# AER-RC/RRTMG_LW

Measured on AMD Instinct MI355X. Metric: columns/sec, 72-layer profiles, higher is better.
Workload: dtype f64 (transmittance / tfn codes and their LDS table f32); 1 GPU; 1000000 synthetic 72-layer columns, config 'cloudy' (icld=2: rtrnmr max-random overlap, idrv=0), sharded 1x1000000; ncol_total=1000000, nlay=72, columns_per_gpu=1000000, parallelism=columns/1, gather=none, kdata=stand-in (real k-data absent from the reference mount), sweeps=production

## Files before the change

rrtmg_lw_amd/csrc/driver.hip:

```cpp
#include <hip/hip_runtime.h>
#include <cstdlib>
#include <sched.h>

#include <algorithm>
#include <array>
#include <atomic>
#include <cstdint>
#include <cstdarg>
#include <mutex>
#include <string>
#include <chrono>
#include <condition_variable>
#include <functional>
#include <map>
#include <thread>
#include <type_traits>
#include <vector>

#include "../../include/rrtmg_lw_hip.h"
#include "kernels.hip"
#include "mtjump.hpp"
#include "hostrows.hpp"
#include "owned.hpp"

// ... 336 lines not shown

int launches_ok()
{
    const hipError_t e = hipGetLastError();
    if (e != hipSuccess) return fail(RRTMG_LW_HIP_EHIP, "kernel launch failed: %s", hipGetErrorString(e));
    return 0;
}

#ifdef RRLW_TUNE
constexpr bool TUNING = true;
#else
constexpr bool TUNING = false;
#endif
constexpr bool sweepc_exists(int phase, bool ddt) { return !ddt || (!TUNING && phase != 1); }
constexpr bool sweepc_ddt(int phase, int idrv) { return idrv == 1 && phase != 1; }
constexpr bool sweepz_exists(int mode, bool ddt) { return !TUNING || (mode == 2 && !ddt); }
constexpr bool layer_exists(bool gcm, int cloud) { return TUNING ? gcm && cloud == 1 : gcm || cloud != 3; }

constexpr int EVERY = -1;
template <int... Vs, class F>
int with_const(int v, F &&f)
{
    int rc = 0;
    bool hit = false;
    ((((v == Vs || v == EVERY) && rc == 0) ? (void)(hit = true, rc = f(std::integral_constant<int, Vs>{})) : (void)0), ...);
    return hit ? rc : fail(RRTMG_LW_HIP_EARG, "internal: no kernel instantiation for %d", v);
}

struct KernelName { char s[24]; };
constexpr KernelName sweep_name(char family, int nq, int x, bool spec)
{
    KernelName n{};
    int k = 0;
    for (const char *p = "k_sweep"; *p; p++) n.s[k++] = *p;
    n.s[k++] = family; n.s[k++] = '<'; n.s[k++] = (char)('0' + nq); n.s[k++] = ','; n.s[k++] = (char)('0' + x);
    if (spec) for (const char *p = ",spec"; *p; p++) n.s[k++] = *p;
    n.s[k++] = '>';
    return n;
}
template <int Q, int PH, bool I, bool SPEC>
struct SweepC {
    static constexpr KernelName name = sweep_name('c', Q, PH, SPEC);
    static constexpr int nt = sweepc_nt(Q, PH);
    static constexpr auto kernel() { return &k_sweepc<Q, PH, I, nt, SPEC>; }
    static int nsb(int nbands) { return sweepc_nsb(Q, PH, I, nbands); }
    static int lds_bytes(int wnb, int nsb) { return sweepc_lds_bytes(PH, I, wnb, nsb, nt); }
};
template <int Q, int M, bool I, bool SPEC>
struct SweepZ {
    static constexpr KernelName name = sweep_name('z', Q, M, SPEC);
    static constexpr int nt = sweepz_nt(Q);
    static constexpr auto kernel() { return &k_sweepz<Q, M, I, SPEC>; }
    static int nsb(int nbands) { return sweepz_nsb(Q, nbands, I); }
    static int lds_bytes(int wnb, int nsb) { return sweepz_lds_bytes(wnb, nsb, nt, I); }
};
template <class F>
int sweepc_dispatch(int nq, int phase, int ddt, int spec, F &&f)
{
    return with_const<1, 2, 3, 4>(nq, [&](auto Q) { return with_const<0, 1, 2>(phase, [&](auto PH) {
           return with_const<0, 1>(ddt, [&](auto I) { return with_const<0, 1>(spec, [&](auto S) {
               if constexpr (sweepc_exists(decltype(PH)::value, decltype(I)::value != 0))
                   return f(SweepC<decltype(Q)::value, decltype(PH)::value, decltype(I)::value != 0, decltype(S)::value != 0>{});
               else return ddt == EVERY ? 0 : fail(RRTMG_LW_HIP_EARG, "internal: no such k_sweepc");
           }); }); }); });
}
template <class F>
int sweepz_dispatch(int nq, int mode, int ddt, int spec, F &&f)
{
    return with_const<1, 2, 3, 4>(nq, [&](auto Q) { return with_const<1, 2, 3, 4>(mode, [&](auto M) {
           return with_const<0, 1>(ddt, [&](auto I) { return with_const<0, 1>(spec, [&](auto S) {
               if constexpr (sweepz_exists(decltype(M)::value, decltype(I)::value != 0))
                   return f(SweepZ<decltype(Q)::value, decltype(M)::value, decltype(I)::value != 0, decltype(S)::value != 0>{});
               else return ddt == EVERY ? 0 : fail(RRTMG_LW_HIP_EARG, "internal: no such k_sweepz");
           }); }); }); });
}

constexpr int N1_LDS_MAX = 160 * 1024;
int ensure_sweep_attrs()
{
    if (G.sweep_attrs) return 0;
    const auto raise = [](auto K) { HIP_TRY(hipFuncSetAttribute((const void *)K.kernel(), hipFuncAttributeMaxDynamicSharedMemorySize, SWEEPC_LDS_MAX)); return 0; };
    if (int rc = sweepc_dispatch(EVERY, EVERY, EVERY, EVERY, raise)) return rc;
    if (int rc = sweepz_dispatch(EVERY, EVERY, EVERY, EVERY, raise)) return rc;
    HIP_TRY(hipFuncSetAttribute((const void *)k_flux<false>, hipFuncAttributeMaxDynamicSharedMemorySize, FLUX_LDS_BYTES));
    HIP_TRY(hipFuncSetAttribute((const void *)k_flux<true>, hipFuncAttributeMaxDynamicSharedMemorySize, FLUX_LDS_BYTES));
#ifndef RRLW_TUNE
    HIP_TRY(hipFuncSetAttribute((const void *)k_n1<false>, hipFuncAttributeMaxDynamicSharedMemorySize, N1_LDS_MAX));
#endif
    G.sweep_attrs = true;
    return 0;
}

struct SweepGroups { int n = 0; int nb[NGROUP_MAX]; unsigned long long bands[NGROUP_MAX]; int gq[NGROUP_MAX]; };
bool make_groups(int mode, int idrv, int istart, int iend, SweepGroups &fg)
{
    unsigned long long lists[5] = {0, 0, 0, 0, 0};
    int nbs[5] = {0, 0, 0, 0, 0};
    for (int nq = 1; nq <= 4; nq++)
        for (int B = 1; B <= NBND; B++)
            if (band_nquad(B) == nq && B >= istart && B <= iend) lists[nq] |= (unsigned long long)(B - 1) << (4 * nbs[nq]++);
    fg.n = 0;
    for (int nq = 4; nq >= 1; nq--) {
        const int zcap = sweepz_group_cap(nq, idrv == 1);
        const int cap = std::max(1, std::min(sweepc_group_cap(nq), mode != 0 ? zcap : 99));
        for (int k0 = 0; k0 < nbs[nq]; k0 += cap) {
            if (fg.n >= NGROUP_MAX) return false;
            const int nbg = std::min(cap, nbs[nq] - k0);
            fg.nb[fg.n] = nbg;
            fg.bands[fg.n] = (lists[nq] >> (4 * k0)) & (nbg >= 16 ? ~0ull : ((1ull << (4 * nbg)) - 1ull));
            fg.gq[fg.n++] = nq;
        }
    }
    return true;
}

void graphs_clear();
int g_split_max = []() { const char *e = getenv("RRTMG_LW_SPLIT_MAX"); return e ? std::max(0, atoi(e)) : 768; }();
int ensure_workspace(int nlay, int ncolb, bool cloud, bool mc = false, int idrv = 1, int mode = -1)
{
    SweepGroups fgw;
    int groups = NGROUP_MAX;
    if (mode >= 0 && make_groups(mode, idrv, 1, NBND, fgw)) groups = fgw.n;
    const bool gdp = idrv == 1, efcl = cloud && (mode < 0 || mode == 1 || mode == 3), ovl = cloud && (mode < 0 || mode == 2);
    const size_t split_cols = ncolb <= g_split_max ? (size_t)NBND * align_up((size_t)ncolb, 64) : 0;
    const State::WsShape &have = G.ws;
    if (G.ws_buf && have.nlay == nlay && have.ncolb >= ncolb && (have.cloud || !cloud) && (have.mc || !mc) && (have.two_scr || !G.split_sweep) &&
        have.groups >= groups && have.slabcols >= split_cols && (have.gdp || !gdp) && (have.efcl || !efcl) && (have.ovl || !ovl)) return 0;
    if (G.ws_buf) { HIP_TRY(hipDeviceSynchronize()); graphs_clear(); if (int rc = drop(G.ws_buf, "workspace")) return rc; }
    const bool same = have.nlay == nlay;
    ncolb = std::max(ncolb, same ? have.ncolb : 0);
    cloud = cloud || have.cloud || mc;
    mc = mc || have.mc;
    const int ng = std::max(groups, have.groups);
    const bool want_gdp = gdp || have.gdp, want_efcl = efcl || have.efcl, want_ovl = ovl || have.ovl;
    const size_t n = (size_t)ncolb, L = (size_t)nlay;
    const size_t slabcols = std::max((size_t)ng * n, (size_t)NBND * align_up(std::min(n, (size_t)std::max(g_split_max, 0)), 64));
    struct Item { void **p; size_t bytes; };
    Workspace &W = G.W;
    W = Workspace{};
    std::vector<Item> items = {
        {(void **)&W.gdn1, slabcols * (L + 1) * sizeof(double)},
        {(void **)&W.gup1, slabcols * (L + 1) * sizeof(double)},
        {(void **)&W.gup, slabcols * (L + 1) * sizeof(Part2)},
        {(void **)&W.gdn, slabcols * (L + 1) * sizeof(Part2)},
    };
    if (want_gdp) items.push_back({(void **)&W.gdp, slabcols * (L + 1) * sizeof(Part2)});
    const bool two_scr = G.split_sweep;
    G.scrset[1] = State::ScrSet{};
    for (int k = 0; k < (two_scr ? 2 : 1); k++) {
        State::ScrSet &ss = G.scrset[k];
        ss = State::ScrSet{};
        items.push_back({(void **)&ss.scr[S_CODE], (size_t)NQUAD * L * n * CODE_BYTES});
        items.push_back({(void **)&ss.fw, (size_t)NFW * L * n * sizeof(unsigned)});
        if (cloud) items.push_back({(void **)&ss.scr[S_CODET], (size_t)NQUAD * L * n * CODE_BYTES});
    }
    for (auto &ps : G.prep) {
        ps = State::PrepSet{};
        items.push_back({(void **)&ps.percol, (size_t)NPERCOL * n * 8});
        items.push_back({(void **)&ps.laytrop, n * 4});
        items.push_back({(void **)&ps.ncbands, n * 4});
        items.push_back({(void **)&ps.cflag, (L + 2) * n * 4});
        const size_t nblk = (n + 63) / 64, nslot = (size_t)sort_slots((int)nblk);
        items.push_back({(void **)&ps.btop, nblk * 4});
        items.push_back({(void **)&ps.hblk, nblk * 4});
        items.push_back({(void **)&ps.order, nslot * 4});
        items.push_back({(void **)&ps.hgrp, (nslot / SORT_GROUP) * 4});
        items.push_back({(void **)&ps.bbot, nblk * 4});
        items.push_back({(void **)&ps.hbot, (nslot / SORT_GROUP) * 4});
// ... 187 lines not shown
    sa.tlev = GCM ? g.tlev : c.tz;
    if (GCM && out.uflxs) { sa.uflxs = out.uflxs; sa.dflxs = out.dflxs; sa.uflxcs = out.uflxcs; sa.dflxcs = out.dflxcs; }
    return sa;
}

template <bool GCM>
int run_sweep(hipStream_t s, const Workspace &Wk_, const Batch &b, const GcmIn &g, const ColIn &c, const FluxOut &out, int sset = 0)
{
    Workspace Wk = Wk_;
    const int nb = b.nb;
    const size_t pcb_split = align_up((size_t)nb, 64);
    const bool split = nb <= g_split_max && (size_t)NBND * pcb_split <= G.ws.slabcols && pcb_split <= (size_t)Wk.ncolb;
    Wk.pcb = split ? (int)pcb_split : Wk.ncolb;
    if (int rc = ensure_sweep_attrs()) return rc;
    const bool fan = G.sweep_fanout;
    State::SweepSet &SS = G.swset[sset];
    if (fan) {
        if (int rc = ensure_sweep_set(sset)) return rc;
        HIP_TRY(hipEventRecord(SS.go.get(), s));
        for (int k = 0; k < 3; k++) HIP_TRY(hipStreamWaitEvent(SS.q[k].get(), SS.go.get(), 0));
    }
    SweepArgs sa = sweep_args<GCM>(b, g, c, out);
    const bool spec = sa.uflxs != nullptr;
#ifndef RRLW_TUNE
    if (G.n1 && b.mode == 0 && GCM && b.istart == 1 && b.iend == 16 && b.idrv == 0 && !spec && n1_lds_bytes(b.nlay) <= N1_LDS_MAX) {
        const dim3 ngrid((nb + N1_WAVES - 1) / N1_WAVES), nblock(64 * N1_WAVES);
        LAUNCH_LDS("k_n1", (k_n1<false>), ngrid, nblock, n1_lds_bytes(b.nlay), s, G.D, Wk, sa, out, g.plev);
        return launches_ok();
    }
#endif
    sa.split = split ? 1 : 0;
    const bool cfree = g_clear_groups && b.mode != 0 && !one_sweep(nb, b.mode);
    sa.cfree = cfree ? 1 : 0;
    SweepGroups fg;
    if (!make_groups(b.mode, b.idrv, b.istart, b.iend, fg)) return fail(RRTMG_LW_HIP_EARG, "internal: more than %d sweep groups", NGROUP_MAX);
    if ((!split && fg.n > G.ws.groups) || (b.idrv == 1 && !G.ws.gdp)) return fail(RRTMG_LW_HIP_EARG, "internal: workspace holds %d band groups, the call needs %d", G.ws.groups, fg.n);
    int slab0[NGROUP_MAX];
    unsigned long long gsz = 0ull;
    { int sl = 0; for (int gi = 0; gi < fg.n; gi++) { slab0[gi] = sl; const int n = split ? fg.nb[gi] : 1; gsz |= (unsigned long long)n << (4 * gi); sl += n; } }
    hipStream_t gs = s;
    const auto launch = [&](auto K) {
        using Kn = decltype(K);
        const int wnb = split ? 1 : sa.nbands;
        const int nsb = split ? 1 : Kn::nsb(sa.nbands);
        sa.ncb = (nb + 64 * nsb - 1) / (64 * nsb);
        const dim3 sgrid((unsigned)sa.ncb, split ? sa.nbands : 1), sblock(64, wnb * Kn::nt, nsb);
        LAUNCH_LDS(Kn::name.s, Kn::kernel(), sgrid, sblock, Kn::lds_bytes(wnb, nsb), gs, G.D, Wk, sa);
        return 0;
    };
    const auto sweepc = [&](int nq, int phase) {
        if (TUNING && b.idrv == 1) return fail(RRTMG_LW_HIP_EARG, "tuning build: idrv = 0 only");
        return sweepc_dispatch(nq, phase, sweepc_ddt(phase, b.idrv), spec, launch);
    };
    const auto sweepz = [&](int nq) {
        const int zmode = b.mode == 1 ? 1 : b.mode == 3 ? (b.mc ? 3 : 4) : 2;
        if (!sweepz_exists(zmode, false)) return fail(RRTMG_LW_HIP_EARG, "tuning build: rtrnmr only");
        if (!sweepz_exists(zmode, b.idrv == 1)) return fail(RRTMG_LW_HIP_EARG, "tuning build: idrv = 0 only");
        return sweepz_dispatch(nq, zmode, b.idrv == 1, spec, launch);
    };
    for (int phase = 0; phase < 3; phase++) {
        if (b.mode == 0 && phase != 0) continue;
        if (phase != 1 && one_sweep(nb, b.mode)) continue;
        for (int gi = 0; gi < fg.n; gi++) {
            const int nq = fg.gq[gi];
            sa.bands = fg.bands[gi];
            sa.nbands = fg.nb[gi];
            sa.group = slab0[gi];
            gs = (fan && nq < 4) ? SS.q[3 - nq].get() : s;
            int rc = 0;
            if (phase == 1) rc = sweepz(nq);
            else if (b.mode == 0) rc = TUNING ? fail(RRTMG_LW_HIP_EARG, "tuning build: cloudy calls only") : sweepc(nq, 0);
            else if (phase == 0) { rc = sweepc(nq, 1); if (rc == 0 && cfree) rc = sweepc(nq, 0); }
            else rc = sweepc(nq, 2);
            if (rc) return rc;
        }
    }
    if (fan) {
        for (int k = 0; k < 3; k++) {
            HIP_TRY(hipEventRecord(SS.done[k].get(), SS.q[k].get()));
            HIP_TRY(hipStreamWaitEvent(s, SS.done[k].get(), 0));
        }
    }
    {
        const dim3 wgrid((nb + COLSORT_WIN - 1) / COLSORT_WIN, (b.nlay + 1 + FLUX_LV - 1) / FLUX_LV), wblock(COLSORT_WIN, FLUX_TY);
        const double *pz = GCM ? g.plev : c.pz;
        if (b.idrv == 1) LAUNCH_LDS("k_flux", (k_flux<true>), wgrid, wblock, FLUX_LDS_BYTES, s, G.D, Wk, out, pz, nb, b.col0, b.nct, b.mode == 0 ? 1 : 0, fg.n, gsz, cfree ? 1 : 0);
        else LAUNCH_LDS("k_flux", (k_flux<false>), wgrid, wblock, FLUX_LDS_BYTES, s, G.D, Wk, out, pz, nb, b.col0, b.nct, b.mode == 0 ? 1 : 0, fg.n, gsz, cfree ? 1 : 0);
    }
    return launches_ok();
}


template <bool GCM>
int run_batch(hipStream_t s, const Batch &b, const GcmIn &g, const ColIn &c, const FluxOut &out)
{
    const Workspace Wk = ws_for(0, use_colsort(GCM, b.mode, b.nb) && !b.mc);
    if (int rc = run_prep<GCM>(s, Wk, b, g, c)) return rc;
    if (int rc = run_layer<GCM>(s, Wk, b, g, c)) return rc;
    return run_sweep<GCM>(s, Wk, b, g, c, out);
}

int ensure_optics_ws(int nlay, int ncolb)
{
    if (G.opt_buf && G.opt_nlay == nlay && G.opt_ncolb >= ncolb) return 0;
    if (int rc = drop(G.opt_buf, "gas-optics workspace")) return rc;
    ncolb = std::max(ncolb, G.opt_nlay == nlay ? G.opt_ncolb : 0);
    const size_t n = (size_t)ncolb, L = (size_t)nlay;
    const size_t b_pc = align_up((size_t)NPERCOL * n * 8, 256), b_lt = align_up(n * 4, 256);
    const size_t b_wide = align_up((2 + ((n + LAYER_BLOCK - 1) / LAYER_BLOCK) * L) * 4, 256);
    if (int rc = grow(G.opt_buf, b_pc + b_lt + b_wide, b_pc + b_lt + b_wide, "gas-optics workspace")) return rc;
    G.opt_percol = G.opt_buf.as<double>();
    G.opt_laytrop = (int *)(G.opt_buf.as<char>() + b_pc);
    G.opt_wide = (int *)(G.opt_buf.as<char>() + b_pc + b_lt);
    HIP_TRY(hipMemset(G.opt_wide, 0, 8));
    G.opt_nlay = nlay;
    G.opt_ncolb = ncolb;
    return 0;
}

template <bool GCM>
int run_optics(hipStream_t s, const Batch &b, const GcmIn &g, const ColIn &c, const OptOut &o)
{
    Workspace W{};
    W.ncolb = G.opt_ncolb; W.pcb = G.opt_ncolb; W.nlay = b.nlay; W.err = G.d_err.as<int>();
    W.percol = G.opt_percol; W.laytrop = G.opt_laytrop;
    W.wide = GCM && HAVE_WIDE && g_wide_window ? G.opt_wide : nullptr;
    LAUNCH("k_colprep", (k_colprep<GCM>), dim3((b.nb + 63) / 64), dim3(64), s, G.D, W, g, c, b.nb, b.col0, b.nct, b.idrv, 1, 0);
    const LayerArgs la = layer_args(b, nullptr);
    const unsigned gx = (b.nb + LAYER_BLOCK - 1) / LAYER_BLOCK;
    if (W.wide) HIP_TRY(hipMemsetAsync(W.wide, 0, sizeof(int), s));
    LAUNCH("k_optics", (k_optics<GCM, 0>), dim3(gx, b.nlay, la.nparts), dim3(LAYER_BLOCK), s, G.D, W, g, c, la, o);
    if constexpr (GCM && HAVE_WIDE) {
        if (W.wide) LAUNCH("k_optics<wide>", (k_optics<true, 1>), dim3(gx * b.nlay, la.nparts), dim3(LAYER_BLOCK), s, G.D, W, g, c, la, o);
    }
    return launches_ok();
}

int check_optics(int idrv, const OptOut &o)
{
    if (!o.taug || !o.fracs) return fail(RRTMG_LW_HIP_EARG, "gas optics: taug and fracs are required");
    if (idrv == 1 && !o.dplankbnd) return fail(RRTMG_LW_HIP_EARG, "gas optics: idrv=1 needs dplankbnd_dt");
    return 0;
}

int ensure_pipeline()
{
    if (G.aux) return 0;
    Event *const ev[] = {&G.ev_in, &G.ev_last, &G.ev_fork, &G.ev_join, &G.ev_ready[0], &G.ev_layer[0], &G.ev_done[0], &G.ev_ready[1], &G.ev_layer[1], &G.ev_done[1]};
    int rc = 0;
    for (Event *e : ev) if (rc == 0) rc = make_event(*e);
    if (rc == 0) rc = make_stream(G.aux, 0, 0);
    if (rc != 0) for (Event *e : ev) (void)e->reset();
    return rc;
}

int launch_kiss(hipStream_t s, const Workspace &Wk, int ncol, int col0, int nb, int nlay, int icld, int permuteseed, const SubcolIn &in);

int g_graph_max = []() { const char *e = getenv("RRTMG_LW_GRAPH_MAX"); return e ? std::max(0, atoi(e)) : 16384; }();
constexpr size_t GRAPH_CACHE = 8;
void graphs_clear()
{
    G.graphs.clear();
}
template <class T> void key_put(std::vector<unsigned char> &k, const T &v)
{
    const unsigned char *p = reinterpret_cast<const unsigned char *>(&v);
    k.insert(k.end(), p, p + sizeof(T));
}

struct KissGen { bool on; int icld, permuteseed; const double *alpha; };

int run_pipelined(hipStream_t s, const Batch &call, const GcmIn &g, const FluxOut &out, KissGen gen = KissGen{false, 0, 0, nullptr})
{
    if (int rc = ensure_pipeline()) return rc;
    const int ncol = call.nct, nlay = call.nlay, mode = call.mode, idrv = call.idrv;
    const McIn *const mc = call.mc;
    const int nbmax = balanced_batch(ncol, eff_batch(nlay));
    const bool single = ncol <= nbmax && !(G.split_sweep && G.cu_layer > 0);
    const hipStream_t aux = single ? s : G.aux.get();
    ColIn c{};
    const bool split = G.split_sweep && G.ws.two_scr && !(mode == 3 && mc);
    const bool part = split && G.cu_layer > 0;
    if (part && !G.lay_m) {
        if (int rc = make_stream(G.lay_u, 0, 0)) return rc;
        if (int rc = make_stream(G.lay_m, 0, G.cu_layer)) return rc;
    }
    if (G.ev_last_valid) HIP_TRY(hipStreamWaitEvent(s, G.ev_last.get(), 0));
    State::GraphEnt *gent = nullptr;
    bool capture = false;
    if (single && !split && !gen.on && !mc && !G.profile && !G.n1 && ncol <= g_graph_max) {
        std::vector<unsigned char> key;
        key_put(key, ncol); key_put(key, nlay); key_put(key, mode); key_put(key, idrv); key_put(key, call.inflag); key_put(key, call.iceflag); key_put(key, call.liqflag);
        const double *gp[] = {g.play, g.plev, g.tlay, g.tlev, g.tsfc, g.h2ovmr, g.o3vmr, g.co2vmr, g.ch4vmr, g.n2ovmr, g.o2vmr, g.cfc11vmr, g.cfc12vmr,
                              g.cfc22vmr, g.ccl4vmr, g.emis, g.cldfr, g.taucld, g.cicewp, g.cliqwp, g.reice, g.reliq, g.tauaer, g.tauctot,
                              out.uflx, out.dflx, out.hr, out.uflxc, out.dflxc, out.hrc, out.duflx_dt, out.duflxc_dt, out.fnet, out.fnetc,
                              out.uflxs, out.dflxs, out.uflxcs, out.dflxcs};
        key_put(key, gp);
        key_put(key, G.init_gen); key_put(key, G.device);
        key_put(key, G.ws_buf.get()); key_put(key, G.ws_buf.bytes()); key_put(key, g_colsort); key_put(key, g_colsort_min); key_put(key, g_colsort_clear); key_put(key, g_clear_groups); key_put(key, g_one_sweep_max);
        key_put(key, g_wide_window); key_put(key, g_layer_split); key_put(key, g_prep_fork); key_put(key, G.sweep_fanout); key_put(key, eff_batch(nlay)); key_put(key, g_split_max);
        for (auto &e : G.graphs) if (e.key == key) { gent = &e; break; }
        if (!gent) {
            if (G.graphs.size() >= GRAPH_CACHE) {
                size_t old = 0;
                for (size_t j = 1; j < G.graphs.size(); j++) if (G.graphs[j].used < G.graphs[old].used) old = j;
                G.graphs.erase(G.graphs.begin() + (long)old);
            }
            G.graphs.emplace_back();
            gent = &G.graphs.back();
            gent->key = key;
        }
        gent->used = ++G.graph_clock;
        if (gent->exec) {
            HIP_TRY(hipGraphLaunch(gent->exec.get(), s));
            G.graph_replays++;
            HIP_TRY(hipEventRecord(G.ev_last.get(), s));
            G.ev_last_valid = true;
            return 0;
        }
        capture = gent->seen >= 1 && !gent->failed;
        gent->seen++;
        if (capture && !G.cap) { if (int rc = make_stream(G.cap, 0, 0)) return rc; }
    }
    const hipStream_t s_call = s;
    if (capture) {
        if (hipStreamBeginCapture(G.cap.get(), hipStreamCaptureModeThreadLocal) != hipSuccess) { (void)hipGetLastError(); capture = false; gent->failed = true; }
        else s = G.cap.get();
    }
    const hipStream_t aux_ = capture ? s : aux;
    if (!single) {
        HIP_TRY(hipEventRecord(G.ev_in.get(), s));
        HIP_TRY(hipStreamWaitEvent(aux, G.ev_in.get(), 0));
    }
    int i = 0, rc_cap = 0;
    Batch b = call;
    for (int col0 = 0; col0 < ncol; col0 += nbmax, i++) {
        const int nb = std::min(nbmax, ncol - col0), k = i & 1;
        b.nb = nb; b.col0 = col0;
        const Workspace Wk = ws_for(k, use_colsort(true, mode, nb) && !mc);
        if (i >= 2) HIP_TRY(hipStreamWaitEvent(aux, G.ev_done[k].get(), 0));
        if (capture) {
            rc_cap = run_prep<true>(s, Wk, b, g, c, g_prep_fork ? G.aux.get() : nullptr);
            if (rc_cap == 0) rc_cap = run_layer<true>(s, Wk, b, g, c);
            if (rc_cap == 0) rc_cap = run_sweep<true>(s, Wk, b, g, c, out);
            continue;
        }
        if (int rc = run_prep<true>(aux, Wk, b, g, c, single && g_prep_fork ? G.aux.get() : nullptr)) return rc;
        if (gen.on) {
            if (int rc = launch_kiss(aux, Wk, ncol, col0, nb, nlay, gen.icld, gen.permuteseed, SubcolIn{g.play, g.cldfr, gen.alpha})) return rc;
        }
        if (!single) HIP_TRY(hipEventRecord(G.ev_ready[k].get(), aux));
        if (!part && !single) HIP_TRY(hipStreamWaitEvent(s, G.ev_ready[k].get(), 0));
        if (split) {
            const bool last = col0 + nbmax >= ncol;
            hipStream_t sl = s;
            int sset = 0;
            if (part) { sl = i == 0 ? G.lay_u.get() : G.lay_m.get(); sset = last ? 0 : 1; }
            if (int rc = ensure_sweep_set(sset)) return rc;
            const hipStream_t ssm = G.swset[sset].main.get();
            if (part) {
                if (i == 0) HIP_TRY(hipStreamWaitEvent(sl, G.ev_in.get(), 0));
                HIP_TRY(hipStreamWaitEvent(sl, G.ev_ready[k].get(), 0));
                if (i >= 1) HIP_TRY(hipStreamWaitEvent(sl, G.ev_layer[(i - 1) & 1].get(), 0));
            }
            if (i >= 2) HIP_TRY(hipStreamWaitEvent(sl, G.ev_done[k].get(), 0));
            if (int rc = run_layer<true>(sl, Wk, b, g, c)) return rc;
            HIP_TRY(hipEventRecord(G.ev_layer[k].get(), sl));
            HIP_TRY(hipStreamWaitEvent(ssm, G.ev_layer[k].get(), 0));
            if (part && i >= 1) HIP_TRY(hipStreamWaitEvent(ssm, G.ev_done[(i - 1) & 1].get(), 0));
            if (int rc = run_sweep<true>(ssm, Wk, b, g, c, out, sset)) return rc;
            HIP_TRY(hipEventRecord(G.ev_done[k].get(), ssm));
        } else {
            if (int rc = run_layer<true>(s, Wk, b, g, c)) return rc;
            if (int rc = run_sweep<true>(s, Wk, b, g, c, out)) return rc;
            HIP_TRY(hipEventRecord(G.ev_done[k].get(), s));
        }
    }
    if (capture) {
        (void)aux_;
        Graph graph;
        const hipError_t ce = hipStreamEndCapture(G.cap.get(), graph.slot());
        s = s_call;
        if (rc_cap != 0) { gent->failed = true; return rc_cap; }
        hipGraphExec_t exec = nullptr;
        if (ce != hipSuccess || !graph || hipGraphInstantiate(&exec, graph.get(), nullptr, nullptr, 0) != hipSuccess) {
            (void)hipGetLastError();
            graph.reset();
            gent->failed = true;
            return run_pipelined(s, call, g, out, gen);
        }
        graph.reset();
        *gent->exec.slot() = exec;
        G.graph_captures++;
        HIP_TRY(hipGraphLaunch(gent->exec.get(), s));
    }
    if (split) {
        for (int k = 0; k < std::min(i, 2); k++) HIP_TRY(hipStreamWaitEvent(s, G.ev_done[k].get(), 0));
    }
    HIP_TRY(hipEventRecord(G.ev_last.get(), s));
    G.ev_last_valid = true;
    return 0;
}

int read_physics_error(hipStream_t s)
{
    int code = 0;
    HIP_TRY(hipMemcpyAsync(&code, G.d_err.as<int>(), sizeof(int), hipMemcpyDeviceToHost, s));
    HIP_TRY(hipStreamSynchronize(s));
    if (code != 0) {
        int zero = 0;
        HIP_TRY(hipMemcpy(G.d_err.as<int>(), &zero, sizeof(int), hipMemcpyHostToDevice));
        return fail(RRTMG_LW_HIP_EPHYSICS, "%s", physics_message(code));
    }
    return 0;
}

int ensure_stage(size_t bytes)
{
    return grow(G.stage_buf, bytes, bytes, "host-entry staging");
}

int check_mcica_build()
{
    return 0;
}

int check_common(int ncol, int nlay)
{
    if (!G.init) return fail(RRTMG_LW_HIP_ENOTINIT, "rrtmg_lw_hip_init has not been called");
    if (ncol < 1 || nlay < 1 || nlay > 603) return fail(RRTMG_LW_HIP_EARG, "bad dimensions ncol=%d nlay=%d", ncol, nlay);
    return 0;
}

int check_spec(const FluxOut &o)
{
    if (!o.uflxs || !o.dflxs) return fail(RRTMG_LW_HIP_EARG, "spectral entry: uflxs and dflxs are required");
    if (!o.uflxcs != !o.dflxcs) return fail(RRTMG_LW_HIP_EARG, "spectral entry: uflxcs and dflxcs must be both null or both set");
    return 0;
}
int check_call(const CallDesc &d, const FluxOut &out)
{
    if (int rc = check_common(d.ncol, d.nlay)) return rc;
    if (d.spectral) if (int rc = check_spec(out)) return rc;
    if (!d.icld) return fail(RRTMG_LW_HIP_EARG, "icld is null");
    if (*d.icld < 0 || *d.icld > 3) *d.icld = 2;
    if (d.idrv == 1 && (!out.duflx_dt || !out.duflxc_dt)) return fail(RRTMG_LW_HIP_EARG, "idrv=1 needs duflx_dt and duflxc_dt");
    return 0;
}

struct HostIn {
    const double *h; size_t inner, rows; double *d;
    bool pinned = false;
    const double *src = nullptr; size_t src_ncol = 0, src_col0 = 0; bool src_pinned = false;
    const unsigned char *skip = nullptr;
    const unsigned char *known = nullptr;
    const uint64_t *known_bits = nullptr;
// ... 2608 lines not shown
```

rrtmg_lw_amd/csrc/kernels.hip:

```cpp
#include <hip/hip_runtime.h>
#include "kissjump.hpp"

#ifdef RRLW_TUNE
#define RRLW_BF_TUNE 1u
#else
#define RRLW_BF_TUNE 0u
#endif
#ifdef RRLW_G256
#define RRLW_BF_G256 8u
#else
#define RRLW_BF_G256 0u
#endif
#if defined(RRLW_LAYER_BLOCK) || defined(RRLW_STAGE_DOUBLES) || defined(RRLW_LAYER_WAVES) || defined(RRLW_LOAD_CHUNK) || defined(RRLW_MINOR_WIN) || \
    defined(RRLW_COLSORT_WIN) || defined(RRLW_SWEEPC_P0) || defined(RRLW_SWEEPC_P2D) || defined(RRLW_SWEEPC_WAVES_CAP) || defined(RRLW_SWEEPC_CODES) || \
    defined(RRLW_SWEEPZ_WAVES_G1) || defined(RRLW_SWEEPZ_WAVES_IDRV) || defined(RRLW_LAYER_STAMPS) || \
    defined(RRLW_DBG_DUMP)
#define RRLW_BF_GEOMETRY 16u
#else
#define RRLW_BF_GEOMETRY 0u
#endif

#include <algorithm>
#include <type_traits>
#include <utility>
// ... 3430 lines not shown
        unsigned w = 0x10000000u;
        if (lower ? m_lo_bin : m_up_bin) w = W.fw[((size_t)m_fwslot * nlay + (lev - 1)) * ncb + col];
        const int r0 = clampi((lower ? 0 : m_base_up) + (int)(w >> 28) - 1, 0, 14);
        const double fpl = (double)(w & 0x0fffffffu) * (1.0 / 268435456.0);
        const double *tp = s_pl[mb];
        const double blay = planck_at(tp, tp, tl);
        const double *tq = (alt && mb == 15) ? T.stat + T.sl.totplk16 : tp;
        const double dpl = planck_at(tp, tq, tz) - blay;
        __builtin_amdgcn_wave_barrier();
        if (lane < 16) { s_pk[4 * mb] = blay; s_pk[4 * mb + 1] = dpl; s_pk[4 * mb + 2] = fpl; s_pk[4 * mb + 3] = (double)r0; }
        __builtin_amdgcn_fence(__ATOMIC_RELEASE, "wavefront");
        __builtin_amdgcn_wave_barrier();
    };
    auto wave_sum = [&](double v) -> double {
#pragma unroll
        for (int o = 32; o >= 1; o >>= 1) v += __shfl_xor(v, o, 64);
        return v;
    };
    double rad[NP1];
#pragma unroll
    for (int p = 0; p < NP1; p++) rad[p] = 0.0;
    auto level = [&](int lev) -> double {
        double part = 0.0;
#pragma unroll
        for (int p = 0; p < NP1; p++) {
            const scr_t cj = ok[p] ? codes[coff[p] + (size_t)(lev - 1) * ncb * 4] : (scr_t)0;
            double atr, tfn;
            decode(cj, s_lut[code_index(cj)], atr, tfn);
            const int b = bnd[p];
            const double blay = s_pk[4 * b], dpl = s_pk[4 * b + 1], fpl = s_pk[4 * b + 2];
            const int r0 = (int)s_pk[4 * b + 3];
            const double f0 = s_fr[b][r0][gi[p]], f1 = s_fr[b][r0 + 1][gi[p]];
            const double fr = f0 + fpl * (f1 - f0);
            const double bb = fr * (blay + tfn * dpl);
            rad[p] = rad[p] + (bb - rad[p]) * atr;
            part += wt[p] * rad[p];
        }
        return wave_sum(part);
    };
    if (lane == 0) s_dn[nlay] = 0.0;
    for (int lev = nlay; lev >= 1; lev--) {
        publish(lev, lev - 1, false);
        const double f = level(lev);
        if (lane == 0) s_dn[lev - 1] = f * T.fluxfac;
    }
    {
        publish(1, 0, false);
        double part = 0.0;
#pragma unroll
        for (int p = 0; p < NP1; p++) {
            const int b = bnd[p];
            const double fpl = s_pk[4 * b + 2];
            const int r0 = (int)s_pk[4 * b + 3];
            const double f0 = s_fr[b][r0][gi[p]], f1 = s_fr[b][r0 + 1][gi[p]];
            const double fr = f0 + fpl * (f1 - f0);
            const double reflect = 1. - a.emis[gc + (size_t)nct * b];
            const double pb = W.percol[(size_t)(PC_PLANKBND + b) * ncb + col];
            rad[p] = fr * pb + reflect * rad[p];
            part += wt[p] * rad[p];
        }
        const double f = wave_sum(part);
        if (lane == 0) s_up[0] = f * T.fluxfac;
    }
    for (int lev = 1; lev <= nlay; lev++) {
        publish(lev, lev, false);
        const double f = level(lev);
        if (lane == 0) s_up[lev] = f * T.fluxfac;
    }
    for (int l0 = 0; l0 <= nlay; l0 += 64) {
        const int lev = l0 + lane;
        if (lev <= nlay) {
            const size_t o = gc + (size_t)nct * lev;
            const double u = s_up[lev], d = s_dn[lev];
            out.uflx[o] = u; out.dflx[o] = d; out.uflxc[o] = u; out.dflxc[o] = d;
            if (out.fnet) { out.fnet[o] = u - d; out.fnetc[o] = u - d; }
            if (lev < nlay) {
                const double h = T.heatfac * ((u - d) - (s_up[lev + 1] - s_dn[lev + 1])) / (pz[o] - pz[o + nct]);
                out.hr[o] = h; out.hrc[o] = h;
            }
        }
    }
}

constexpr int FLUX_LV = 8, FLUX_TY = 4;
static_assert(COLSORT_WIN * FLUX_TY <= 1024, "k_flux: a window x FLUX_TY threads");
constexpr int FLUX_LDS_BYTES = (FLUX_LV + 1) * 4 * COLSORT_WIN * 8;
template <bool IDRV>
__global__ __launch_bounds__(COLSORT_WIN * FLUX_TY) void k_flux(DevTables T, Workspace W, FluxOut out, const double *pz, int ncol, int col0, int nct,
                                                                int clear_from_total, int ngroups, unsigned long long gsz, int clear_groups)
{
    constexpr int NV = 4, NL = (FLUX_LV + FLUX_TY) / FLUX_TY;
    extern __shared__ __align__(16) unsigned char smem_f[];
    double (*s_v)[NV][COLSORT_WIN] = reinterpret_cast<double (*)[NV][COLSORT_WIN]>(smem_f);
    double kdu[IDRV ? NL : 1], kduc[IDRV ? NL : 1];
    const int t = threadIdx.x, ty = threadIdx.y, w0 = blockIdx.x * COLSORT_WIN;
    const int slot = w0 + t, col = w0 + t;
    const bool son = slot < ncol, con = col < ncol;
    const int nlay = W.nlay, lev0 = blockIdx.y * FLUX_LV;
    const size_t ncb = W.ncolb, gc = (size_t)col0 + col;
    const int dst = son ? pcol(W, slot) - w0 : t;
    const int ltop = (son && !clear_from_total) ? W.hblk[slot >> 6] : 0;
    const bool up1 = clear_from_total != 0 || (clear_groups != 0 && son && ltop == 0);
#pragma unroll
    for (int k = 0; k < NL; k++) {
        const int lc = ty + k * FLUX_TY, lev = lev0 + lc;
        if constexpr (IDRV) { kdu[k] = 0.0; kduc[k] = 0.0; }
        if (lc <= FLUX_LV && son && lev <= nlay) {
            const bool dn1 = clear_from_total || lev >= ltop;
            double u = 0.0, d = 0.0, uc = 0.0, dc = 0.0, du = 0.0, duc = 0.0;
            const size_t pcb = (size_t)W.pcb;
            int slab = 0;
            for (int g = 0; g < ngroups; g++) {
                const int n = (int)((gsz >> (4 * g)) & 15ull);
                Part2 su{0.0, 0.0}, sd{0.0, 0.0}, sq{0.0, 0.0};
                for (int q = 0; q < n; q++, slab++) {
                    const size_t go = ((size_t)slab * (nlay + 1) + lev) * pcb + slot;
                    Part2 tu, td, tq{0.0, 0.0};
                    if (dn1) { td.a = W.gdn1[go]; td.b = td.a; } else td = W.gdn[go];
                    if (up1) { tu.a = W.gup1[go]; tu.b = tu.a; } else tu = W.gup[go];
                    if constexpr (IDRV) tq = W.gdp[go];
                    if (q == 0) { su = tu; sd = td; sq = tq; }
                    else { su.a = su.a + tu.a; su.b = su.b + tu.b; sd.a = sd.a + td.a; sd.b = sd.b + td.b; sq.a = sq.a + tq.a; sq.b = sq.b + tq.b; }
                }
                u = u + su.a; uc = uc + su.b;
                d = d + sd.a; dc = dc + sd.b;
                du = du + sq.a; duc = duc + sq.b;
            }
            u = u * T.fluxfac; d = d * T.fluxfac;
            if (clear_from_total) { uc = u; dc = d; duc = du; }
            else { uc = uc * T.fluxfac; dc = dc * T.fluxfac; }
            s_v[lc][0][dst] = u; s_v[lc][1][dst] = d; s_v[lc][2][dst] = uc; s_v[lc][3][dst] = dc;
            if constexpr (IDRV) { kdu[k] = du; kduc[k] = duc; }
        }
    }
    __syncthreads();
    for (int lc = ty; lc < FLUX_LV; lc += FLUX_TY) {
        const int lev = lev0 + lc;
        if (con && lev <= nlay) {
            const double u = s_v[lc][0][t], d = s_v[lc][1][t], uc = s_v[lc][2][t], dc = s_v[lc][3][t];
            const size_t o = gc + (size_t)nct * lev;
            out.uflx[o] = u; out.dflx[o] = d; out.uflxc[o] = uc; out.dflxc[o] = dc;
            if (out.fnet) { out.fnet[o] = u - d; out.fnetc[o] = uc - dc; }
            if (lev < nlay) {
                const double net = u - d, netc = uc - dc;
                const double above = s_v[lc + 1][0][t] - s_v[lc + 1][1][t], abovec = s_v[lc + 1][2][t] - s_v[lc + 1][3][t];
                const double dp = pz[o] - pz[o + (size_t)nct];
                out.hr[o] = T.heatfac * (net - above) / dp;
                out.hrc[o] = T.heatfac * (netc - abovec) / dp;
            }
        }
    }
    if constexpr (IDRV) {
        __syncthreads();
#pragma unroll
        for (int k = 0; k < NL; k++) {
            const int lc = ty + k * FLUX_TY, lev = lev0 + lc;
            if (lc < FLUX_LV && son && lev <= nlay) { s_v[lc][0][dst] = kdu[k]; s_v[lc][1][dst] = kduc[k]; }
        }
        __syncthreads();
        for (int lc = ty; lc < FLUX_LV; lc += FLUX_TY) {
            const int lev = lev0 + lc;
            if (con && lev <= nlay) {
                const size_t o = gc + (size_t)nct * lev;
                out.duflx_dt[o] = s_v[lc][0][t]; out.duflxc_dt[o] = s_v[lc][1][t];
            }
        }
    }
}

__global__ __launch_bounds__(256) void k_calibrate(const double2 *__restrict__ in, double2 *__restrict__ out, size_t n)
{
    const size_t i = (size_t)blockIdx.x * blockDim.x + threadIdx.x;
    if (i < n) { double2 v = in[i]; v.x += 1.0; out[i] = v; }
}

struct AdjustSet { const void *u, *d, *du; void *ua, *hr; };
struct AdjustArgs {
    const void *plev, *dtsfc;
    AdjustSet s[2];
    unsigned long long ncol;
    int nlay, chunk;
    int vec;
    double heatfac;
};
template <class R, int V> struct AdjustVec { typedef R type __attribute__((ext_vector_type(V))); };
template <class R, int V>
__device__ __forceinline__ void adjust_load(const void *p, size_t at, double (&x)[V])
{
    if constexpr (V == 1) x[0] = (double)static_cast<const R *>(p)[at];
    else {
        const typename AdjustVec<R, V>::type v = *reinterpret_cast<const typename AdjustVec<R, V>::type *>(static_cast<const R *>(p) + at);
#pragma unroll
        for (int j = 0; j < V; j++) x[j] = (double)v[j];
    }
}
template <class R, int V>
__device__ __forceinline__ void adjust_store(void *p, size_t at, const double (&x)[V])
{
    if constexpr (V == 1) static_cast<R *>(p)[at] = (R)x[0];
    else {
        typename AdjustVec<R, V>::type v;
#pragma unroll
        for (int j = 0; j < V; j++) v[j] = (R)x[j];
        *reinterpret_cast<typename AdjustVec<R, V>::type *>(static_cast<R *>(p) + at) = v;
    }
}
__device__ __forceinline__ double adjust_up(double u, double du, double dt)
{
#pragma clang fp contract(off)
    const double prod = du * dt;
    return u + prod;
}

template <class R, int V, bool TOP, int NS>
__global__ __launch_bounds__(256) void k_adjust_cf(AdjustArgs a)
{
#pragma clang fp contract(off)
    const size_t n = (size_t)a.ncol, c = ((size_t)blockIdx.x * 256 + threadIdx.x) * V;
    if (c >= n) return;
    const int nlay = a.nlay, k0 = (int)blockIdx.y * a.chunk, k1 = min(nlay, k0 + a.chunk);
    double dt[V], pb[V], nb[NS][V];
    adjust_load<R, V>(a.dtsfc, c, dt);
#pragma unroll 2
    for (int k = k0; k <= k1; k++) {
        const size_t at = (size_t)(TOP ? nlay - k : k) * n + c;
        const bool mine = k < k1 || k1 == nlay;
        double p[V], net[NS][V];
        adjust_load<R, V>(a.plev, at, p);
#pragma unroll
        for (int s = 0; s < NS; s++) {
            double u[V], d[V], du[V];
            adjust_load<R, V>(a.s[s].u, at, u);
            adjust_load<R, V>(a.s[s].d, at, d);
            adjust_load<R, V>(a.s[s].du, at, du);
#pragma unroll
            for (int j = 0; j < V; j++) { u[j] = adjust_up(u[j], du[j], dt[j]); net[s][j] = u[j] - d[j]; }
            if (mine) adjust_store<R, V>(a.s[s].ua, at, u);
        }
        if (k > k0) {
            const size_t ah = (size_t)(TOP ? nlay - k : k - 1) * n + c;
#pragma unroll
            for (int s = 0; s < NS; s++) {
                double h[V];
#pragma unroll
                for (int j = 0; j < V; j++) h[j] = a.heatfac * (nb[s][j] - net[s][j]) / (pb[j] - p[j]);
                adjust_store<R, V>(a.s[s].hr, ah, h);
            }
        }
// ... 287 lines not shown
```

Baseline: 17.69 million columns/s.

## Restructure flux kernel into per-column level marching and prefetch next batch prep

The k_flux kernel drops its 2D thread layout and per-block level tiles. Each thread now walks a chunk of levels for one column, carrying the previous level's net flux and pressure in registers to compute heating rates. A fast path with software-prefetched loads handles the common four-single-slab group layout, and the LDS permutation exchange only happens when columns were moved. Separately, the host loop issues the next batch's prep on the aux stream between the layer and sweep launches, so prep can overlap the current sweep. The costs are one recomputed overlap level per chunk and a per-level barrier on moved windows.

```diff
diff --git a/rrtmg_lw_amd/csrc/driver.hip b/rrtmg_lw_amd/csrc/driver.hip
--- a/rrtmg_lw_amd/csrc/driver.hip
+++ b/rrtmg_lw_amd/csrc/driver.hip
@@ -442,8 +442,6 @@
     const auto raise = [](auto K) { HIP_TRY(hipFuncSetAttribute((const void *)K.kernel(), hipFuncAttributeMaxDynamicSharedMemorySize, SWEEPC_LDS_MAX)); return 0; };
     if (int rc = sweepc_dispatch(EVERY, EVERY, EVERY, EVERY, raise)) return rc;
     if (int rc = sweepz_dispatch(EVERY, EVERY, EVERY, EVERY, raise)) return rc;
-    HIP_TRY(hipFuncSetAttribute((const void *)k_flux<false>, hipFuncAttributeMaxDynamicSharedMemorySize, FLUX_LDS_BYTES));
-    HIP_TRY(hipFuncSetAttribute((const void *)k_flux<true>, hipFuncAttributeMaxDynamicSharedMemorySize, FLUX_LDS_BYTES));
 #ifndef RRLW_TUNE
     HIP_TRY(hipFuncSetAttribute((const void *)k_n1<false>, hipFuncAttributeMaxDynamicSharedMemorySize, N1_LDS_MAX));
 #endif
@@ -797,10 +795,10 @@
         }
     }
     {
-        const dim3 wgrid((nb + COLSORT_WIN - 1) / COLSORT_WIN, (b.nlay + 1 + FLUX_LV - 1) / FLUX_LV), wblock(COLSORT_WIN, FLUX_TY);
+        const dim3 wgrid((nb + COLSORT_WIN - 1) / COLSORT_WIN, (b.nlay + 1 + FLUX_CH - 1) / FLUX_CH), wblock(COLSORT_WIN);
         const double *pz = GCM ? g.plev : c.pz;
-        if (b.idrv == 1) LAUNCH_LDS("k_flux", (k_flux<true>), wgrid, wblock, FLUX_LDS_BYTES, s, G.D, Wk, out, pz, nb, b.col0, b.nct, b.mode == 0 ? 1 : 0, fg.n, gsz, cfree ? 1 : 0);
-        else LAUNCH_LDS("k_flux", (k_flux<false>), wgrid, wblock, FLUX_LDS_BYTES, s, G.D, Wk, out, pz, nb, b.col0, b.nct, b.mode == 0 ? 1 : 0, fg.n, gsz, cfree ? 1 : 0);
+        if (b.idrv == 1) LAUNCH("k_flux", (k_flux<true>), wgrid, wblock, s, G.D, Wk, out, pz, nb, b.col0, b.nct, b.mode == 0 ? 1 : 0, fg.n, gsz, cfree ? 1 : 0);
+        else LAUNCH("k_flux", (k_flux<false>), wgrid, wblock, s, G.D, Wk, out, pz, nb, b.col0, b.nct, b.mode == 0 ? 1 : 0, fg.n, gsz, cfree ? 1 : 0);
     }
     return launches_ok();
 }
@@ -949,22 +947,31 @@
     }
     int i = 0, rc_cap = 0;
     Batch b = call;
+    const auto prep = [&](int j) -> int {
+        Batch bj = call;
+        bj.col0 = j * nbmax; bj.nb = std::min(nbmax, ncol - bj.col0);
+        const int kj = j & 1;
+        const Workspace Wj = ws_for(kj, use_colsort(true, mode, bj.nb) && !mc);
+        if (j >= 2) HIP_TRY(hipStreamWaitEvent(aux, G.ev_done[kj].get(), 0));
+        if (int rc = run_prep<true>(aux, Wj, bj, g, c, single && g_prep_fork ? G.aux.get() : nullptr)) return rc;
+        if (gen.on) {
+            if (int rc = launch_kiss(aux, Wj, ncol, bj.col0, bj.nb, nlay, gen.icld, gen.permuteseed, SubcolIn{g.play, g.cldfr, gen.alpha})) return rc;
+        }
+        if (!single) HIP_TRY(hipEventRecord(G.ev_ready[kj].get(), aux));
+        return 0;
+    };
+    const bool ahead = !single && !split && !capture && !gen.on;
     for (int col0 = 0; col0 < ncol; col0 += nbmax, i++) {
         const int nb = std::min(nbmax, ncol - col0), k = i & 1;
         b.nb = nb; b.col0 = col0;
         const Workspace Wk = ws_for(k, use_colsort(true, mode, nb) && !mc);
-        if (i >= 2) HIP_TRY(hipStreamWaitEvent(aux, G.ev_done[k].get(), 0));
         if (capture) {
             rc_cap = run_prep<true>(s, Wk, b, g, c, g_prep_fork ? G.aux.get() : nullptr);
             if (rc_cap == 0) rc_cap = run_layer<true>(s, Wk, b, g, c);
             if (rc_cap == 0) rc_cap = run_sweep<true>(s, Wk, b, g, c, out);
             continue;
         }
-        if (int rc = run_prep<true>(aux, Wk, b, g, c, single && g_prep_fork ? G.aux.get() : nullptr)) return rc;
-        if (gen.on) {
-            if (int rc = launch_kiss(aux, Wk, ncol, col0, nb, nlay, gen.icld, gen.permuteseed, SubcolIn{g.play, g.cldfr, gen.alpha})) return rc;
-        }
-        if (!single) HIP_TRY(hipEventRecord(G.ev_ready[k].get(), aux));
+        if (!ahead || i == 0) { if (int rc = prep(i)) return rc; }
         if (!part && !single) HIP_TRY(hipStreamWaitEvent(s, G.ev_ready[k].get(), 0));
         if (split) {
             const bool last = col0 + nbmax >= ncol;
@@ -987,6 +994,7 @@
             HIP_TRY(hipEventRecord(G.ev_done[k].get(), ssm));
         } else {
             if (int rc = run_layer<true>(s, Wk, b, g, c)) return rc;
+            if (ahead && col0 + nbmax < ncol) { if (int rc = prep(i + 1)) return rc; }
             if (int rc = run_sweep<true>(s, Wk, b, g, c, out)) return rc;
             HIP_TRY(hipEventRecord(G.ev_done[k].get(), s));
         }
diff --git a/rrtmg_lw_amd/csrc/kernels.hip b/rrtmg_lw_amd/csrc/kernels.hip
--- a/rrtmg_lw_amd/csrc/kernels.hip
+++ b/rrtmg_lw_amd/csrc/kernels.hip
@@ -3536,39 +3536,72 @@
     }
 }
 
-constexpr int FLUX_LV = 8, FLUX_TY = 4;
-static_assert(COLSORT_WIN * FLUX_TY <= 1024, "k_flux: a window x FLUX_TY threads");
-constexpr int FLUX_LDS_BYTES = (FLUX_LV + 1) * 4 * COLSORT_WIN * 8;
+constexpr int FLUX_CH = 18;
+constexpr int FLUX_NG = 4;
+constexpr unsigned long long FLUX_GSZ1 = 0x1111ull;
+template <bool IDRV> struct FluxRaw { Part2 u[FLUX_NG], d[FLUX_NG], q[IDRV ? FLUX_NG : 1]; };
+struct FluxVal { double u, d, uc, dc, du, duc; };
+constexpr int flux_lds_bytes(bool idrv) { return 2 * (idrv ? 6 : 4) * COLSORT_WIN * 8; }
 template <bool IDRV>
-__global__ __launch_bounds__(COLSORT_WIN * FLUX_TY) void k_flux(DevTables T, Workspace W, FluxOut out, const double *pz, int ncol, int col0, int nct,
-                                                                int clear_from_total, int ngroups, unsigned long long gsz, int clear_groups)
-{
-    constexpr int NV = 4, NL = (FLUX_LV + FLUX_TY) / FLUX_TY;
-    extern __shared__ __align__(16) unsigned char smem_f[];
-    double (*s_v)[NV][COLSORT_WIN] = reinterpret_cast<double (*)[NV][COLSORT_WIN]>(smem_f);
-    double kdu[IDRV ? NL : 1], kduc[IDRV ? NL : 1];
-    const int t = threadIdx.x, ty = threadIdx.y, w0 = blockIdx.x * COLSORT_WIN;
-    const int slot = w0 + t, col = w0 + t;
-    const bool son = slot < ncol, con = col < ncol;
-    const int nlay = W.nlay, lev0 = blockIdx.y * FLUX_LV;
-    const size_t ncb = W.ncolb, gc = (size_t)col0 + col;
-    const int dst = son ? pcol(W, slot) - w0 : t;
-    const int ltop = (son && !clear_from_total) ? W.hblk[slot >> 6] : 0;
-    const bool up1 = clear_from_total != 0 || (clear_groups != 0 && son && ltop == 0);
-#pragma unroll
-    for (int k = 0; k < NL; k++) {
-        const int lc = ty + k * FLUX_TY, lev = lev0 + lc;
-        if constexpr (IDRV) { kdu[k] = 0.0; kduc[k] = 0.0; }
-        if (lc <= FLUX_LV && son && lev <= nlay) {
+__global__ __launch_bounds__(COLSORT_WIN) void k_flux(DevTables T, Workspace W, FluxOut out, const double *pz, int ncol, int col0, int nct,
+                                                      int clear_from_total, int ngroups, unsigned long long gsz, int clear_groups)
+{
+    constexpr int NV = IDRV ? 6 : 4;
+    __shared__ double s_v[2][NV][COLSORT_WIN];
+    static_assert(sizeof(s_v) == flux_lds_bytes(IDRV), "k_flux: the exchange tile");
+    const int t = threadIdx.x, w0 = blockIdx.x * COLSORT_WIN;
+    const int slot = w0 + t;
+    const bool on = slot < ncol;
+    const int nlay = W.nlay;
+    const int k0 = blockIdx.y * FLUX_CH, k1 = min(nlay, k0 + FLUX_CH - 1), kf = max(k0 - 1, 0);
+    const size_t gc = (size_t)col0 + slot;
+    const bool moved = pmoved(W, w0);
+    const int dst = (moved && on) ? W.perm[slot] - w0 : t;
+    const int ltop = __builtin_amdgcn_readfirstlane((on && !clear_from_total) ? W.hblk[slot >> 6] : 0);
+    const bool up1 = clear_from_total != 0 || (clear_groups != 0 && ltop == 0);
+    const size_t pcb = (size_t)W.pcb, nlev = (size_t)nlay + 1;
+    const auto load = [&](int lev, FluxRaw<IDRV> &r) {
+        if (!on) return;
+        const size_t g0 = (size_t)lev * pcb + slot, gs = nlev * pcb;
+        if (clear_from_total || lev >= ltop) {
+#pragma unroll
+            for (int g = 0; g < FLUX_NG; g++) { r.d[g].a = W.gdn1[g0 + g * gs]; r.d[g].b = r.d[g].a; }
+        } else {
+#pragma unroll
+            for (int g = 0; g < FLUX_NG; g++) r.d[g] = W.gdn[g0 + g * gs];
+        }
+        if (up1) {
+#pragma unroll
+            for (int g = 0; g < FLUX_NG; g++) { r.u[g].a = W.gup1[g0 + g * gs]; r.u[g].b = r.u[g].a; }
+        } else {
+#pragma unroll
+            for (int g = 0; g < FLUX_NG; g++) r.u[g] = W.gup[g0 + g * gs];
+        }
+        if constexpr (IDRV) {
+#pragma unroll
+            for (int g = 0; g < FLUX_NG; g++) r.q[g] = W.gdp[g0 + g * gs];
+        }
+    };
+    const auto sum = [&](const FluxRaw<IDRV> &r) -> FluxVal {
+        double u = 0.0, d = 0.0, uc = 0.0, dc = 0.0, du = 0.0, duc = 0.0;
+#pragma unroll
+        for (int g = 0; g < FLUX_NG; g++) {
+            u = u + r.u[g].a; uc = uc + r.u[g].b;
+            d = d + r.d[g].a; dc = dc + r.d[g].b;
+            if constexpr (IDRV) { du = du + r.q[g].a; duc = duc + r.q[g].b; }
+        }
+        return FluxVal{u, d, uc, dc, du, duc};
+    };
+    const auto sum_list = [&](int lev) -> FluxVal {
+        double u = 0.0, d = 0.0, uc = 0.0, dc = 0.0, du = 0.0, duc = 0.0;
+        if (on) {
             const bool dn1 = clear_from_total || lev >= ltop;
-            double u = 0.0, d = 0.0, uc = 0.0, dc = 0.0, du = 0.0, duc = 0.0;
-            const size_t pcb = (size_t)W.pcb;
             int slab = 0;
             for (int g = 0; g < ngroups; g++) {
                 const int n = (int)((gsz >> (4 * g)) & 15ull);
                 Part2 su{0.0, 0.0}, sd{0.0, 0.0}, sq{0.0, 0.0};
                 for (int q = 0; q < n; q++, slab++) {
-                    const size_t go = ((size_t)slab * (nlay + 1) + lev) * pcb + slot;
+                    const size_t go = ((size_t)slab * nlev + lev) * pcb + slot;
                     Part2 tu, td, tq{0.0, 0.0};
                     if (dn1) { td.a = W.gdn1[go]; td.b = td.a; } else td = W.gdn[go];
                     if (up1) { tu.a = W.gup1[go]; tu.b = tu.a; } else tu = W.gup[go];
@@ -3580,44 +3613,52 @@
                 d = d + sd.a; dc = dc + sd.b;
                 du = du + sq.a; duc = duc + sq.b;
             }
-            u = u * T.fluxfac; d = d * T.fluxfac;
-            if (clear_from_total) { uc = u; dc = d; duc = du; }
-            else { uc = uc * T.fluxfac; dc = dc * T.fluxfac; }
-            s_v[lc][0][dst] = u; s_v[lc][1][dst] = d; s_v[lc][2][dst] = uc; s_v[lc][3][dst] = dc;
-            if constexpr (IDRV) { kdu[k] = du; kduc[k] = duc; }
-        }
-    }
-    __syncthreads();
-    for (int lc = ty; lc < FLUX_LV; lc += FLUX_TY) {
-        const int lev = lev0 + lc;
-        if (con && lev <= nlay) {
-            const double u = s_v[lc][0][t], d = s_v[lc][1][t], uc = s_v[lc][2][t], dc = s_v[lc][3][t];
-            const size_t o = gc + (size_t)nct * lev;
+        }
+        return FluxVal{u, d, uc, dc, du, duc};
+    };
+    double pb = 0.0, nb = 0.0, nbc = 0.0;
+    const auto level = [&](int lev, FluxVal v, double p) {
+        double u = v.u * T.fluxfac, d = v.d * T.fluxfac, uc, dc, du = v.du, duc = v.duc;
+        if (clear_from_total) { uc = u; dc = d; duc = du; }
+        else { uc = v.uc * T.fluxfac; dc = v.dc * T.fluxfac; }
+        if (moved) {
+            double (*s)[COLSORT_WIN] = s_v[lev & 1];
+            s[0][dst] = u; s[1][dst] = d; s[2][dst] = uc; s[3][dst] = dc;
+            if constexpr (IDRV) { s[4][dst] = du; s[5][dst] = duc; }
+            __syncthreads();
+            u = s[0][t]; d = s[1][t]; uc = s[2][t]; dc = s[3][t];
+            if constexpr (IDRV) { du = s[4][t]; duc = s[5][t]; }
+        }
+        if (!on) return;
+        const size_t o = gc + (size_t)nct * lev;
+        const double net = u - d, netc = uc - dc;
+        if (lev >= k0) {
             out.uflx[o] = u; out.dflx[o] = d; out.uflxc[o] = uc; out.dflxc[o] = dc;
             if (out.fnet) { out.fnet[o] = u - d; out.fnetc[o] = uc - dc; }
-            if (lev < nlay) {
-                const double net = u - d, netc = uc - dc;
-                const double above = s_v[lc + 1][0][t] - s_v[lc + 1][1][t], abovec = s_v[lc + 1][2][t] - s_v[lc + 1][3][t];
-                const double dp = pz[o] - pz[o + (size_t)nct];
-                out.hr[o] = T.heatfac * (net - above) / dp;
-                out.hrc[o] = T.heatfac * (netc - abovec) / dp;
-            }
-        }
-    }
-    if constexpr (IDRV) {
-        __syncthreads();
-#pragma unroll
-        for (int k = 0; k < NL; k++) {
-            const int lc = ty + k * FLUX_TY, lev = lev0 + lc;
-            if (lc < FLUX_LV && son && lev <= nlay) { s_v[lc][0][dst] = kdu[k]; s_v[lc][1][dst] = kduc[k]; }
-        }
-        __syncthreads();
-        for (int lc = ty; lc < FLUX_LV; lc += FLUX_TY) {
-            const int lev = lev0 + lc;
-            if (con && lev <= nlay) {
-                const size_t o = gc + (size_t)nct * lev;
-                out.duflx_dt[o] = s_v[lc][0][t]; out.duflxc_dt[o] = s_v[lc][1][t];
-            }
+            if constexpr (IDRV) { out.duflx_dt[o] = du; out.duflxc_dt[o] = duc; }
+        }
+        if (lev > kf) {
+            const double dp = pb - p;
+            out.hr[o - (size_t)nct] = T.heatfac * (nb - net) / dp;
+            out.hrc[o - (size_t)nct] = T.heatfac * (nbc - netc) / dp;
+        }
+        pb = p; nb = net; nbc = netc;
+    };
+    const double *const pzc = pz + gc;
+    double p = on ? pzc[(size_t)nct * kf] : 0.0;
+    if (ngroups == FLUX_NG && gsz == FLUX_GSZ1) {
+        FluxRaw<IDRV> cur{}, nxt{};
+        load(kf, cur);
+        for (int lev = kf; lev <= k1; lev++) {
+            double pn = 0.0;
+            if (lev < k1) { load(lev + 1, nxt); if (on) pn = pzc[(size_t)nct * (lev + 1)]; }
+            level(lev, sum(cur), p);
+            cur = nxt; p = pn;
+        }
+    } else {
+        for (int lev = kf; lev <= k1; lev++) {
+            level(lev, sum_list(lev), p);
+            if (lev < k1 && on) p = pzc[(size_t)nct * (lev + 1)];
         }
     }
 }
```

New measurement: 17.87 million columns/s, median of 6. 1.01x the previous value.
